# leggedrobotics/art_planner

Hardware: NVIDIA H100
Metric: pose-validity checks/s (higher is better)
Workload: dtype f32

## Files before the change

### art_planner_b200/csrc/artp_capi.cu

```cuda
#include <cassert>
#include <climits>
#include <cmath>
#include <cstdlib>
#include <cstring>
#include <type_traits>
#include <vector>

#include "artp_internal.h"
#include "artp_kernels.cuh"
#include "artp_tiles.cuh"

using namespace artp_api;

namespace {

thread_local std::string g_create_error;

__global__ void reverse_columns_kernel(const float* __restrict__ layer, float* __restrict__ H, int nx, int nz, int pitch) {
  const size_t total = (size_t)pitch * nz;
  for (size_t i = blockIdx.x * (size_t)blockDim.x + threadIdx.x; i < total; i += (size_t)gridDim.x * blockDim.x) {
    const int z = (int)(i / pitch), x = (int)(i - (size_t)z * pitch);
    H[i] = (x < nx) ? layer[x + (size_t)(nz - 1 - z) * nx] * 1.0f + 0.0f : 0.0f;
  }
}

__global__ void build_level_kernel(const float* __restrict__ H, const float2* __restrict__ prevT,
                                   const unsigned char* __restrict__ prevNF, const unsigned char* __restrict__ mergeable,
                                   float2* __restrict__ T, unsigned char* __restrict__ NF, int nx, int nz, int pitch, int half) {
  const size_t total = (size_t)pitch * nz;
  for (size_t i = blockIdx.x * (size_t)blockDim.x + threadIdx.x; i < total; i += (size_t)gridDim.x * blockDim.x) {
    const int z = (int)(i / pitch), x = (int)(i - (size_t)z * pitch);
    if (x >= nx) { T[i] = make_float2(0.f, 0.f); NF[i] = 0; continue; }
    const int x2 = min(x + half, nx - 1), z2 = min(z + half, nz - 1);
    const size_t id[4] = {(size_t)z * pitch + x, (size_t)z * pitch + x2, (size_t)z2 * pitch + x, (size_t)z2 * pitch + x2};
    float mx = -CUDART_INF_F, mn = CUDART_INF_F;
    unsigned char nf = 0;
#pragma unroll
    for (int q = 0; q < 4; ++q) {
      if (prevT) {
        const float2 v = prevT[id[q]];
        mx = fmaxf(mx, v.x); mn = fminf(mn, v.y); nf |= prevNF[id[q]];
      } else {
        const float h = H[id[q]];
        mx = fmaxf(mx, h);
        if (fabsf(h) < CUDART_INF_F) mn = fminf(mn, h); else nf |= 1;
        nf |= mergeable[id[q]];
      }
    }
    T[i] = make_float2(mx, mn);
    NF[i] = nf;
  }
}

__global__ void build_codes_kernel(const float2* __restrict__ T, const unsigned char* __restrict__ NF, uint32_t* __restrict__ C,
                                   size_t n, float base, float step) {
  const float top = artp::code_dec(base, step, artp::kCodeMax);
  for (size_t i = blockIdx.x * (size_t)blockDim.x + threadIdx.x; i < n; i += (size_t)gridDim.x * blockDim.x) {
    const float2 v = T[i];
    uint32_t cM = 0, cm = artp::kCodeNone;
    if (v.x > top) cM = artp::kCodeNone;
    else if (v.x > -CUDART_INF_F) {
      uint32_t lo = 1, hi = artp::kCodeMax;
      while (lo < hi) {
        const uint32_t mid = (lo + hi) >> 1;
        if (artp::code_dec(base, step, mid) >= v.x) hi = mid; else lo = mid + 1;
      }
      cM = lo;
    }
    if (v.y <= top) {
      uint32_t lo = 0, hi = artp::kCodeMax;
      while (lo < hi) {
        const uint32_t mid = (lo + hi + 1) >> 1;
        if (artp::code_dec(base, step, mid) <= v.y) lo = mid; else hi = mid - 1;
      }
      cm = lo;
    }
    C[i] = artp::code_word(cM, cm, NF[i] & 3u);
  }
}

void code_scale(const float* layer, size_t n, float& base, float& step) {
  float lo = HUGE_VALF, hi = -HUGE_VALF;
  for (size_t i = 0; i < n; ++i) {
    const float v = layer[i] * 1.0f + 0.0f;
    if (std::fabs(v) < HUGE_VALF) { lo = std::min(lo, v); hi = std::max(hi, v); }
  }
  base = lo <= hi ? lo : 0.0f;
  int e = -126;
  while (e < 127 && artp::code_dec(base, std::ldexp(1.0f, e), artp::kCodeMax) < hi) ++e;
  step = std::ldexp(1.0f, e);
}

struct PlaneSlot { unsigned long long key; uint32_t lo, hi; };
constexpr unsigned long long kEmptyKey = ~0ull;
__device__ __forceinline__ unsigned long long plane_key(int kx, int kz, int kd) {
  return ((unsigned long long)(uint32_t)(kx & 0xffff) << 48) | ((unsigned long long)(uint32_t)(kz & 0xffff) << 32) | (uint32_t)kd;
}
__device__ __forceinline__ uint32_t plane_slot_hash(unsigned long long k) {
  k ^= k >> 33; k *= 0xff51afd7ed558ccdull; k ^= k >> 33; k *= 0xc4ceb9fe1a85ec53ull; k ^= k >> 33;
  return (uint32_t)k;
}
__global__ void plane_table_clear_kernel(PlaneSlot* tab, size_t cap) {
  for (size_t i = blockIdx.x * (size_t)blockDim.x + threadIdx.x; i < cap; i += (size_t)gridDim.x * blockDim.x) {
    tab[i].key = kEmptyKey; tab[i].lo = 0xffffffffu; tab[i].hi = 0u;
  }
}
__device__ __forceinline__ bool cell_tri_plane(const artp::Field& f, int x, int x_off, int z, int u, float pl[4]) {
  float hA, hB, hC, hD;
  artp::load_cell(f, x, z, hA, hB, hC, hD);
  const bool ok = u == 0 ? (artp::finitef(hA) && artp::finitef(hB) && artp::finitef(hC))
                         : (artp::finitef(hD) && artp::finitef(hB) && artp::finitef(hC));
  if (!ok) return false;
  artp::cell_plane(f, u == 0, x + x_off, z, hA, hB, hC, hD, pl);
  return true;
}
__global__ void plane_table_insert_kernel(const artp::Field f, int x_off, PlaneSlot* tab, uint32_t mask) {
  const size_t ncell = (size_t)(f.nx - 1) * (f.nz - 1);
  for (size_t i = blockIdx.x * (size_t)blockDim.x + threadIdx.x; i < 2 * ncell; i += (size_t)gridDim.x * blockDim.x) {
    const size_t c = i >> 1;
    const int u = (int)(i & 1), z = (int)(c / (f.nx - 1)), x = (int)(c - (size_t)z * (f.nx - 1));
    float pl[4];
    if (!cell_tri_plane(f, x, x_off, z, u, pl)) continue;
    const uint32_t id = (uint32_t)(((size_t)z * f.pitch + x) * 2 + u);
    const unsigned long long key = plane_key(artp::nkey(pl[0]), artp::nkey(pl[2]), artp::dkey(pl[3]));
    uint32_t s = plane_slot_hash(key) & mask;
    for (;;) {
      const unsigned long long old = atomicCAS(&tab[s].key, kEmptyKey, key);
      if (old == kEmptyKey || old == key) {
        if (!(tab[s].lo < id && tab[s].hi > id)) { atomicMin(&tab[s].lo, id); atomicMax(&tab[s].hi, id); }
        break;
      }
      s = (s + 1) & mask;
    }
  }
}
__global__ void plane_table_query_kernel(const artp::Field f, int x_off, const PlaneSlot* __restrict__ tab, uint32_t mask,
                                         unsigned char* __restrict__ mergeable) {
  const size_t ncell = (size_t)(f.nx - 1) * (f.nz - 1);
  for (size_t i = blockIdx.x * (size_t)blockDim.x + threadIdx.x; i < 2 * ncell; i += (size_t)gridDim.x * blockDim.x) {
    const size_t c = i >> 1;
    const int u = (int)(i & 1), z = (int)(c / (f.nx - 1)), x = (int)(c - (size_t)z * (f.nx - 1));
    float pl[4];
    if (!cell_tri_plane(f, x, x_off, z, u, pl)) continue;
    const uint32_t id = (uint32_t)(((size_t)z * f.pitch + x) * 2 + u);
    const float e2 = 2.0f * ARTP_EPS;
    const int kx0 = artp::nkey(pl[0] - e2), kx1 = artp::nkey(pl[0] + e2);
    const int kz0 = artp::nkey(pl[2] - e2), kz1 = artp::nkey(pl[2] + e2);
    const int kd0 = artp::dkey(pl[3] - e2), kd1 = artp::dkey(pl[3] + e2);
    bool dup = false;
    for (int kx = kx0; kx <= kx1 && !dup; ++kx)
      for (int kz = kz0; kz <= kz1 && !dup; ++kz)
        for (int kd = kd0; kd <= kd1 && !dup; ++kd) {
          const unsigned long long key = plane_key(kx, kz, kd);
          uint32_t s = plane_slot_hash(key) & mask;
          for (;;) {
            const unsigned long long k = tab[s].key;
            if (k == kEmptyKey) break;
            if (k == key) { dup = tab[s].lo != id || tab[s].hi != id; break; }
            s = (s + 1) & mask;
          }
        }
    if (dup) mergeable[(size_t)z * f.pitch + x] = 2;
  }
}

__global__ void fill_u8_kernel(uint8_t* p, size_t n, uint8_t v) {
  for (size_t i = blockIdx.x * (size_t)blockDim.x + threadIdx.x; i < n; i += (size_t)gridDim.x * blockDim.x) p[i] = v;
}

constexpr int kCompactBlock = 1024;
template <bool BITS>
__device__ __forceinline__ int mask_at(const uint8_t* __restrict__ valid, size_t i) {
  if (BITS) return (int)((reinterpret_cast<const uint32_t*>(valid)[i >> 5] >> (i & 31)) & 1u);
  return valid[i] != 0;
}
template <bool BITS>
__global__ void compact_count_kernel(const uint8_t* __restrict__ valid, size_t n, uint32_t* __restrict__ counts) {
  const size_t i = (size_t)blockIdx.x * kCompactBlock + threadIdx.x;
  const int v = (i < n) && mask_at<BITS>(valid, i);
  const int c = __syncthreads_count(v);
  if (threadIdx.x == 0) counts[blockIdx.x] = (uint32_t)c;
}
__global__ void compact_scan_kernel(uint32_t* counts, size_t nb, uint32_t* total) {
  __shared__ uint32_t carry;
  __shared__ uint32_t wsum[32];
  if (threadIdx.x == 0) carry = 0;
  __syncthreads();
  for (size_t b0 = 0; b0 < nb; b0 += blockDim.x) {
    const size_t i = b0 + threadIdx.x;
    const uint32_t v = i < nb ? counts[i] : 0u;
    uint32_t x = v;
    const int lane = threadIdx.x & 31, wid = threadIdx.x >> 5;
    for (int o = 1; o < 32; o <<= 1) { const uint32_t y = __shfl_up_sync(0xffffffffu, x, o); if (lane >= o) x += y; }
    if (lane == 31) wsum[wid] = x;
    __syncthreads();
    if (wid == 0) {
      uint32_t s = lane < (int)(blockDim.x >> 5) ? wsum[lane] : 0u;
      for (int o = 1; o < 32; o <<= 1) { const uint32_t y = __shfl_up_sync(0xffffffffu, s, o); if (lane >= o) s += y; }
      wsum[lane] = s;
    }
    __syncthreads();
    const uint32_t before = carry + (wid ? wsum[wid - 1] : 0u) + x - v;
    if (i < nb) counts[i] = before;
    __syncthreads();
    if (threadIdx.x == blockDim.x - 1) carry = before + v;
    __syncthreads();
  }
  if (threadIdx.x == 0) *total = carry;
}
template <bool BITS, typename IndexT>
__global__ void compact_scatter_kernel(const uint8_t* __restrict__ valid, size_t n, int64_t base,
                                       const uint32_t* __restrict__ offsets, IndexT* __restrict__ out) {
  __shared__ uint32_t wsum[32];
  const size_t i = (size_t)blockIdx.x * kCompactBlock + threadIdx.x;
  const int v = (i < n) && mask_at<BITS>(valid, i);
  const unsigned bal = __ballot_sync(0xffffffffu, v);
  const int lane = threadIdx.x & 31, wid = threadIdx.x >> 5;
  if (lane == 0) wsum[wid] = __popc(bal);
  __syncthreads();
  if (wid == 0) {
    uint32_t s = wsum[lane];
    for (int o = 1; o < 32; o <<= 1) { const uint32_t y = __shfl_up_sync(0xffffffffu, s, o); if (lane >= o) s += y; }
    wsum[lane] = s;
  }
  __syncthreads();
  if (v) {
    const uint32_t pos = offsets[blockIdx.x] + (wid ? wsum[wid - 1] : 0u) + __popc(bal & ((1u << lane) - 1u));
    out[pos] = (IndexT)(base + (int64_t)i);
  }
}

__global__ void pack_bits_kernel(const uint8_t* __restrict__ valid, size_t n, uint32_t* __restrict__ bits) {
  const size_t words = (n + 31) / 32;
  const size_t warps = ((size_t)gridDim.x * blockDim.x) >> 5, wid = ((size_t)blockIdx.x * blockDim.x + threadIdx.x) >> 5;
  const int lane = threadIdx.x & 31;
  for (size_t w = wid; w < words; w += warps) {
    const size_t i = w * 32 + lane;
    const unsigned bal = __ballot_sync(0xffffffffu, i < n && valid[i] != 0);
    if (lane == 0) bits[w] = bal;
  }
}

constexpr size_t kChunkItems = 1u << 20;

int ensure_queues(Handle* h, size_t n_items) {
  const size_t need = 5 * std::min(n_items, kChunkItems);
  if (h->recs_cap >= need) return ARTP_OK;
  const size_t cap = std::max<size_t>(need, 1u << 16);
  h->recs_cap = 0;
  size_t had[4] = {0, 0, 0, 0};
  int rc;
  TRY(grow(h, h->d_recs, had[0], cap));
  TRY(grow(h, h->d_recs_f, had[1], cap));
  TRY(grow(h, h->d_recs_g, had[2], cap));
  TRY(grow(h, h->d_defer, had[3], cap));
  h->recs_cap = cap;
  return ARTP_OK;
}

struct HostFeed {
  const char* host;
  char* dev;
  size_t bytes_per_item;
  size_t slice_items;
  float schedule[8];
};
constexpr size_t kScheduleItems = 1u << 18;
constexpr int kPipeReachCtasPerSm = 2;

__global__ void close_slice_kernel(const BoxQueues* round, BoxQueues* slices, int i) {
  const BoxQueues prev = i ? slices[i - 1] : BoxQueues{};
  slices[i].group = {round->group.end, prev.group.end};
  slices[i].reach = {round->reach.end, prev.reach.end};
  slices[i].big = {round->big.end, prev.big.end};
}

int launch_classify(Handle* h, artp::Work w, size_t lo, size_t hi, cudaStream_t s) {
  w.item_base = (uint32_t)lo;
  w.n_items = (uint32_t)hi;
  BoxQueues* q = &h->d_ctr->q;
  return launch(h, artp::classify_items_kernel, (unsigned)((hi - lo + artp::kClassifyItems - 1) / artp::kClassifyItems),
                artp::kClassifyItems, 0, s, h->chk, w, h->d_recs, h->d_recs_f, h->group_grid ? h->d_recs_g : nullptr, &q->big.end,
                &q->reach.end, &q->group.end, h->mode == 1);
}

int launch_big_tile(Handle* h, artp::Work w, size_t lo, size_t hi, BoxQueues* q, cudaStream_t s) {
  w.item_base = (uint32_t)lo;
  w.n_items = (uint32_t)hi;
  const int wpc = h->tile_warps[0];
  const unsigned grid = (unsigned)std::min<size_t>((size_t)h->tile_grid[0], (5 * (hi - lo) + wpc - 1) / wpc);
  return launch(h, artp::box_tiles_warp_kernel, grid, wpc * 32, h->tile_smem[0], s, h->chk, h->tile_map[0][0], h->tile_map[0][1],
                h->tile_cfg[0], w, h->d_recs, &q->big.end, &q->big.claim, &h->d_ctr->defer, h->d_defer, 0u, h->mode == 1);
}
int launch_reach_warp(Handle* h, artp::Work w, size_t lo, size_t hi, BoxQueues* q, cudaStream_t s, unsigned reach_cap) {
  if (!h->chk.reach_tw) return ARTP_OK;
  w.item_base = (uint32_t)lo;
  w.n_items = (uint32_t)hi;
  const int wpc = h->tile_warps[1];
  const unsigned grid = (unsigned)std::min<size_t>({(size_t)h->tile_grid[1], (4 * (hi - lo) + wpc - 1) / wpc, reach_cap});
  return launch(h, artp::box_tiles_warp_kernel, grid, wpc * 32, h->tile_smem[1], s, h->chk, h->tile_map[1][1], h->tile_map[1][1],
                h->tile_cfg[1], w, h->d_recs_f, &q->reach.end, &q->reach.claim, &h->d_ctr->defer, h->d_defer, artp::kDeferReachBit,
                h->mode == 1);
}
int launch_reach_groups(Handle* h, artp::Work w, size_t lo, size_t hi, BoxQueues* q, cudaStream_t s, unsigned reach_cap) {
  if (!h->group_grid) return ARTP_OK;
  w.item_base = (uint32_t)lo;
  w.n_items = (uint32_t)hi;
  const unsigned grid = (unsigned)std::min<size_t>({(size_t)h->group_grid, (hi - lo + 7) / 8, reach_cap});
  return launch(h, artp::reach_groups_kernel, grid, artp::kMaxTileWarps * 32, h->group_smem, s, h->chk, h->tile_map[1][1],
                h->tile_cfg[1], w, h->d_recs_g, &q->group.end, &q->group.claim);
}

int launch_grouping(Handle* h, artp::Work w, size_t lo, size_t hi, cudaStream_t s) {
  w.item_base = (uint32_t)lo;
  w.n_items = (uint32_t)hi;
  const unsigned grid = (unsigned)std::min<size_t>((size_t)h->k2_grid, 5 * (hi - lo));
  return launch(h, artp::box_items_block_kernel, grid, artp::kBlockStageThreads, h->k2_smem, s, h->chk, w, h->d_recs, h->d_recs_f,
                &h->d_ctr->defer, h->d_defer, h->k2_tcap, h->d_err);
}

int run_round_device(Handle* h, const artp::Work& w, cudaStream_t s, size_t base, size_t end, bool timed) {
  CU_TRY(h, cudaMemsetAsync(h->d_ctr, 0, sizeof(Counters), s));
  if (timed) CU_TRY(h, cudaEventRecord(h->ev[0], s));
  TRY(launch_classify(h, w, base, end, s));
  if (timed) CU_TRY(h, cudaEventRecord(h->ev[1], s));
  const bool fork = !h->timing && h->chk.reach_tw;
  if (fork) {
    CU_TRY(h, cudaEventRecord(h->slice_ev[0], s));
    CU_TRY(h, cudaStreamWaitEvent(h->box_stream, h->slice_ev[0], 0));
    if (h->group_grid) CU_TRY(h, cudaStreamWaitEvent(h->group_stream, h->slice_ev[0], 0));
  }
  BoxQueues* q = &h->d_ctr->q;
  TRY(launch_big_tile(h, w, base, end, q, s));
  if (timed) CU_TRY(h, cudaEventRecord(h->ev[2], s));
  TRY(launch_reach_warp(h, w, base, end, q, fork ? h->box_stream : s, UINT_MAX));
  if (timed) CU_TRY(h, cudaEventRecord(h->ev[3], s));
  TRY(launch_reach_groups(h, w, base, end, q, fork ? h->group_stream : s, UINT_MAX));
  if (fork) {
    CU_TRY(h, cudaEventRecord(h->box_ev, h->box_stream));
    CU_TRY(h, cudaStreamWaitEvent(s, h->box_ev, 0));
    if (h->group_grid) {
      CU_TRY(h, cudaEventRecord(h->group_ev, h->group_stream));
      CU_TRY(h, cudaStreamWaitEvent(s, h->group_ev, 0));
    }
  }
  if (timed) CU_TRY(h, cudaEventRecord(h->ev[4], s));
  TRY(launch_grouping(h, w, base, end, s));
  if (timed) { CU_TRY(h, cudaEventRecord(h->ev[5], s)); h->ev_valid = true; }
  return ARTP_OK;
}

int run_round_piped(Handle* h, const artp::Work& w, cudaStream_t s, const HostFeed& feed, size_t base, size_t end) {
  size_t cut[kMaxSlices + 1];
  int ncut = 0;
  cut[0] = base;
  if (end - base >= kScheduleItems) {
    double acc = 0.0;
    for (int i = 0; i < 8 && feed.schedule[i] > 0.0f; ++i) {
      acc += feed.schedule[i];
      const size_t c = std::min(end, (base + (size_t)((double)(end - base) * acc) + 127) & ~(size_t)127);
      if (c > cut[ncut]) cut[++ncut] = c;
    }
    if (cut[ncut] != end) cut[++ncut] = end;
  } else {
    for (size_t lo = base; lo < end; lo += feed.slice_items) cut[++ncut] = std::min(end, lo + feed.slice_items);
  }
  assert(ncut <= kMaxSlices);
  CU_TRY(h, cudaMemsetAsync(h->d_ctr, 0, sizeof(Counters), s));
  const unsigned reach_cap = (unsigned)(kPipeReachCtasPerSm * h->sm_count);
  for (int si = 0; si < ncut; ++si) {
    const size_t lo = cut[si], hi = cut[si + 1];
    CU_TRY(h, cudaMemcpyAsync(feed.dev + lo * feed.bytes_per_item, feed.host + lo * feed.bytes_per_item,
                              (hi - lo) * feed.bytes_per_item, cudaMemcpyHostToDevice, h->copy_stream));
    CU_TRY(h, cudaEventRecord(h->copy_ev[si], h->copy_stream));
    CU_TRY(h, cudaStreamWaitEvent(s, h->copy_ev[si], 0));
    TRY(launch_classify(h, w, lo, hi, s));
    TRY(launch(h, close_slice_kernel, 1, 1, 0, s, &h->d_ctr->q, h->d_slices, si));
    CU_TRY(h, cudaEventRecord(h->slice_ev[si], s));
    CU_TRY(h, cudaStreamWaitEvent(h->box_stream, h->slice_ev[si], 0));
    if (h->group_grid) CU_TRY(h, cudaStreamWaitEvent(h->group_stream, h->slice_ev[si], 0));
    TRY(launch_reach_groups(h, w, lo, hi, h->d_slices + si, h->group_stream, reach_cap));
    TRY(launch_reach_warp(h, w, lo, hi, h->d_slices + si, h->box_stream, reach_cap));
    TRY(launch_big_tile(h, w, lo, hi, h->d_slices + si, h->box_stream));
  }
  if (h->group_grid) {
    CU_TRY(h, cudaEventRecord(h->group_ev, h->group_stream));
    CU_TRY(h, cudaStreamWaitEvent(h->box_stream, h->group_ev, 0));
  }
  TRY(launch_grouping(h, w, base, end, h->box_stream));
  CU_TRY(h, cudaEventRecord(h->box_ev, h->box_stream));
  CU_TRY(h, cudaStreamWaitEvent(s, h->box_ev, 0));
  return ARTP_OK;
}

int run_items(Handle* h, artp::Work w, cudaStream_t s, const HostFeed* feed = nullptr) {
  const size_t n_total = w.n_items;
  TRY(ensure_queues(h, n_total));
  for (size_t base = 0; base < n_total; base += kChunkItems) {
    const size_t end = std::min(n_total, base + kChunkItems);
    if (feed && feed->slice_items < end - base && !h->timing) {
      TRY(run_round_piped(h, w, s, *feed, base, end));
    } else {
      if (feed)
        CU_TRY(h, cudaMemcpyAsync(feed->dev + base * feed->bytes_per_item, feed->host + base * feed->bytes_per_item,
                                  (end - base) * feed->bytes_per_item, cudaMemcpyHostToDevice, s));
      TRY(run_round_device(h, w, s, base, end, h->timing && end == n_total));
    }
  }
  h->deferred_unread = true;
  return ARTP_OK;
}

int check_common(Handle* h, size_t n) {
  TRY(require_map(h));
  if (n >= (size_t)0xFFFFFFF0u) { h->err = "too many items for one call"; return ARTP_E_LIMIT; }
  return ARTP_OK;
}

int check_poses_small(Handle* h, const artp::SmallBatch& sb, size_t n, uint8_t* valid, int steps = -1) {
  TRY(host_call_begin(h));
  if (!h->h_small_out) {
    CU_TRY(h, cudaHostAlloc((void**)&h->h_small_out, 64, cudaHostAllocMapped));
    CU_TRY(h, cudaFuncSetAttribute(artp::pose_small_kernel, cudaFuncAttributeMaxDynamicSharedMemorySize, 200 * 1024));
  }
  uint8_t* d_out = nullptr;
  CU_TRY(h, cudaHostGetDevicePointer((void**)&d_out, h->h_small_out, 0));
  TRY(launch(h, artp::pose_small_kernel, (unsigned)n, 256, h->k2_smem, h->stream, h->chk, sb, d_out, h->k2_tcap, h->d_err,
      h->mode == 1, steps));
  const int rc = host_call_end(h, true);
  if (rc == ARTP_E_CUDA) return rc;
  if (steps < 0) {
    std::memcpy(valid, h->h_small_out, n);
  } else {
    const size_t per = (size_t)steps + 1;
    for (size_t e = 0; e < n / per; ++e) {
      uint8_t ok = 1;
      for (size_t j = 0; j < per; ++j) ok &= h->h_small_out[e * per + j];
      valid[e] = ok;
    }
  }
  h->stats.poses_checked += n;
  h->ev_valid = false;
  return rc;
}

template <typename T>
int check_states(Handle* h, const T* d_states, size_t n, uint8_t* d_valid, cudaStream_t s, const HostFeed* feed = nullptr) {
  artp::Work w;
  if constexpr (std::is_same_v<T, float>) w.s2f = d_states; else w.s2 = d_states;
  w.valid = d_valid;
  w.n_items = (uint32_t)n;
  TRY(run_items(h, w, s, feed));
  h->stats.poses_checked += n;
  return ARTP_OK;
}

template <typename T>
int check_poses(Handle* h, const T* states, size_t n, uint8_t* valid, bool on_device, cudaStream_t stream) {
  TRY(check_common(h, n));
  if (n == 0) return ARTP_OK;
  if (!states || !valid) return null_buffer(h);
  if (on_device) {
    CU_TRY(h, cudaSetDevice(h->device));
    ChainScope cs(h, 0, stream);
    if (cs.rc) return cs.rc;
    return check_states(h, states, n, valid, stream);
  }
  if (n <= (size_t)artp::kSmallBatch && !h->timing) {
    artp::SmallBatch sb;
    for (size_t i = 0; i < n * 7; ++i) (&sb.s[0][0])[i] = (double)states[i];
    return check_poses_small(h, sb, n, valid);
  }
  char* r[2];
  TRY(host_call_begin(h, {n * 7 * sizeof(T), n}, r));
  const HostFeed feed = std::is_same_v<T, float>
                            ? HostFeed{(const char*)states, r[0], 7 * sizeof(T), 256 * 1024, {0.08f, 0.17f, 0.25f, 0.25f, 0.25f}}
                            : HostFeed{(const char*)states, r[0], 7 * sizeof(T), 128 * 1024, {0.06f, 0.14f, 0.20f, 0.20f, 0.20f, 0.20f}};
  TRY(check_states(h, (const T*)r[0], n, (uint8_t*)r[1], h->stream, &feed));
  CU_TRY(h, cudaMemcpyAsync(valid, r[1], n, cudaMemcpyDeviceToHost, h->stream));
  return host_call_end(h, true);
}

int motion_items(Handle* h, size_t n, int n_steps) {
  if (n_steps < 0) { h->err = "n_steps < 0"; return ARTP_E_INVALID; }
  return check_common(h, n * ((size_t)n_steps + 1));
}
int check_motions_on(Handle* h, const double* d_s1, const double* d_s2, size_t n, int n_steps, uint8_t* d_valid, cudaStream_t s) {
  TRY(launch(h, fill_u8_kernel, grid_for(h, n, 256, 8), 256, 0, s, d_valid, n, 1));
  const size_t items = n * ((size_t)n_steps + 1);
  artp::Work w;
  w.s1 = d_s1; w.s2 = d_s2; w.valid = d_valid; w.n_items = (uint32_t)items; w.steps = n_steps; w.edge_mode = 1;
  TRY(run_items(h, w, s));
  h->stats.poses_checked += items;
  return ARTP_OK;
}

__global__ void edge_prefix_kernel(const uint8_t* __restrict__ item_valid, const uint32_t* __restrict__ item_off, size_t n,
                                   int32_t* __restrict__ valid_prefix) {
  for (size_t e = blockIdx.x * (size_t)blockDim.x + threadIdx.x; e < n; e += (size_t)gridDim.x * blockDim.x) {
    const uint32_t o0 = item_off[e], o1 = item_off[e + 1];
    uint32_t k = o0;
    while (k < o1 && item_valid[k]) ++k;
    valid_prefix[e] = (int32_t)(k - o0);
  }
}

int check_items_prefix(Handle* h, const double* d_s1, const double* d_s2, size_t n, const uint32_t* d_item_off,
                       size_t total_items, uint8_t* d_item_valid, int32_t* d_valid_prefix, void* stream, int quotient) {
  TRY(check_common(h, total_items));
  if (n == 0) return ARTP_OK;
  if (!d_s1 || !d_s2 || !d_item_off || !d_valid_prefix || (total_items && !d_item_valid)) {
    return null_buffer(h);
  }
  if (n >= 0xFFFFFFFFull) { h->err = "too many edges"; return ARTP_E_INVALID; }
  CU_TRY(h, cudaSetDevice(h->device));
  cudaStream_t s = (cudaStream_t)stream;
  ChainScope cs(h, 0, s);
  if (cs.rc) return cs.rc;
  if (total_items) {
    artp::Work w;
    w.s1 = d_s1; w.s2 = d_s2; w.valid = d_item_valid; w.n_items = (uint32_t)total_items;
    w.item_off = d_item_off; w.n_edges = (uint32_t)n; w.quotient = quotient;
    TRY(run_items(h, w, s));
  }
  TRY(launch(h, edge_prefix_kernel, grid_for(h, n, 256, 8), 256, 0, s, d_item_valid, d_item_off, n, d_valid_prefix));
  h->stats.poses_checked += total_items;
  return ARTP_OK;
}

int check_items_prefix_host(Handle* h, const double* s1, const double* s2, const std::vector<uint32_t>& off, int quotient,
                            int32_t* valid_prefix) {
  const size_t n = off.size() - 1, total = off[n], sb = n * 7 * sizeof(double);
  char* r[5];
  TRY(host_call_begin(h, {sb, sb, (n + 1) * sizeof(uint32_t), n * sizeof(int32_t), total}, r));
  CU_TRY(h, cudaMemcpyAsync(r[0], s1, sb, cudaMemcpyHostToDevice, h->stream));
  CU_TRY(h, cudaMemcpyAsync(r[1], s2, sb, cudaMemcpyHostToDevice, h->stream));
  CU_TRY(h, cudaMemcpyAsync(r[2], off.data(), (n + 1) * sizeof(uint32_t), cudaMemcpyHostToDevice, h->stream));
  TRY(check_items_prefix(h, (const double*)r[0], (const double*)r[1], n, (const uint32_t*)r[2], total, (uint8_t*)r[4],
                         (int32_t*)r[3], h->stream, quotient));
  CU_TRY(h, cudaMemcpyAsync(valid_prefix, r[3], n * sizeof(int32_t), cudaMemcpyDeviceToHost, h->stream));
  return host_call_end(h, true);
}

int pack_valid_bits(Handle* h, const uint8_t* d_valid, size_t n, uint32_t* d_bits, cudaStream_t s) {
  if (n == 0) return ARTP_OK;
  if (!d_valid || !d_bits) return null_buffer(h);
  CU_TRY(h, cudaSetDevice(h->device));
  const size_t words = (n + 31) / 32;
  return launch(h, pack_bits_kernel, grid_for(h, words * 32, 256, 8), 256, 0, s, d_valid, n, d_bits);
}

}

int artp_api::take_sticky_error(Handle* h) {
  if (h->h_err && *(volatile uint32_t*)h->h_err) {
    const uint32_t e = *(volatile uint32_t*)h->h_err;
    *(volatile uint32_t*)h->h_err = 0;
    if (e & 2u) {
      h->err = "a box reached outside this handle's map window (artp_set_map_window: route samples to the shard that holds them, "
               "halo >= box half-diagonal + offsets); affected poses were marked invalid";
      return ARTP_E_WINDOW;
    }
    h->err = "plane-grouping stage overflow: a zone exceeded its shared-memory store; affected poses were marked invalid";
    return ARTP_E_LIMIT;
  }
  return ARTP_OK;
}

int artp_api::check_states_f32(Handle* h, const float* d_states, size_t n, uint8_t* d_valid, cudaStream_t s) {
  return check_states(h, d_states, n, d_valid, s);
}

int artp_api::check_states_cta(Handle* h, const double* d_states, const uint32_t* d_count, const uint32_t* d_stop, size_t max_n,
                               uint8_t* d_valid, cudaStream_t s) {
  if (max_n == 0) return ARTP_OK;
  if (!h->pose_states_smem) {
    CU_TRY(h, cudaFuncSetAttribute(artp::pose_states_kernel, cudaFuncAttributeMaxDynamicSharedMemorySize, 200 * 1024));
    h->pose_states_smem = true;
  }
  TRY(launch(h, artp::pose_states_kernel, (unsigned)max_n, 256, h->k2_smem, s, h->chk, d_states, d_count, d_stop, d_valid,
             h->k2_tcap, h->d_err));
  h->ev_valid = false;
  return ARTP_OK;
}

int artp_api::compact_valid(Handle* h, const uint8_t* d_valid, size_t n, int64_t base, void* d_indices, uint32_t* d_count,
                            cudaStream_t s, bool bits, bool u32) {
  if (n == 0) { CU_TRY(h, cudaMemsetAsync(d_count, 0, sizeof(uint32_t), s)); return ARTP_OK; }
  ChainScope cs(h, 1, s);
  if (cs.rc) return cs.rc;
  const size_t nb = (n + kCompactBlock - 1) / kCompactBlock;
  TRY(grow(h, h->d_block_counts, h->block_counts_cap, nb));
  TRY(bits ? launch(h, compact_count_kernel<true>, (unsigned)nb, kCompactBlock, 0, s, d_valid, n, h->d_block_counts)
           : launch(h, compact_count_kernel<false>, (unsigned)nb, kCompactBlock, 0, s, d_valid, n, h->d_block_counts));
  TRY(launch(h, compact_scan_kernel, 1, 1024, 0, s, h->d_block_counts, nb, d_count));
  if (bits)
    return launch(h, compact_scatter_kernel<true, int64_t>, (unsigned)nb, kCompactBlock, 0, s, d_valid, n, base, h->d_block_counts,
                  (int64_t*)d_indices);
  if (u32)
    return launch(h, compact_scatter_kernel<false, uint32_t>, (unsigned)nb, kCompactBlock, 0, s, d_valid, n, base,
                  h->d_block_counts, (uint32_t*)d_indices);
  return launch(h, compact_scatter_kernel<false, int64_t>, (unsigned)nb, kCompactBlock, 0, s, d_valid, n, base, h->d_block_counts,
                (int64_t*)d_indices);
}

extern "C" {

const char* artp_version(void) { return "artp 0.1 sm_90a"; }

const char* artp_last_error(const artp_handle* hh) {
  if (!hh) return g_create_error.c_str();
  return reinterpret_cast<const Handle*>(hh)->err.c_str();
}

int artp_create(const artp_params* params, artp_handle** out) {
  if (!params || !out) { g_create_error = "null argument"; return ARTP_E_INVALID; }
  *out = nullptr;
  int ndev = 0;
  cudaError_t e = cudaGetDeviceCount(&ndev);
  if (e != cudaSuccess || ndev == 0) {
    g_create_error = std::string("no CUDA device: ") + cudaGetErrorString(e);
    return ARTP_E_CUDA;
  }
  if (params->device < 0 || params->device >= ndev) { g_create_error = "bad device ordinal"; return ARTP_E_INVALID; }
  if (!(params->torso_length > 0 && params->torso_width > 0 && params->torso_height > 0 && params->reach_x > 0 &&
        params->reach_y > 0 && params->reach_z > 0)) {
    g_create_error = "box dimensions must be positive";
    return ARTP_E_INVALID;
  }
  Handle* h = new Handle();
  h->p = *params;
  h->device = params->device;
  auto fail = [&](const char* what, cudaError_t ce) {
    g_create_error = std::string(what) + ": " + cudaGetErrorString(ce);
    artp_destroy(reinterpret_cast<artp_handle*>(h));
    return ARTP_E_CUDA;
  };
  if ((e = cudaSetDevice(h->device)) != cudaSuccess) return fail("cudaSetDevice", e);
  cudaDeviceProp prop;
  if ((e = cudaGetDeviceProperties(&prop, h->device)) != cudaSuccess) return fail("cudaGetDeviceProperties", e);
  h->sm_count = prop.multiProcessorCount;
  cudaFuncAttributes fa;
  if ((e = cudaFuncGetAttributes(&fa, artp::box_tiles_warp_kernel)) != cudaSuccess)
    return fail("no usable kernel image (built for sm_90a)", e);
  for (cudaStream_t* st : {&h->stream, &h->copy_stream, &h->box_stream, &h->group_stream})
    if ((e = cudaStreamCreateWithFlags(st, cudaStreamNonBlocking)) != cudaSuccess) return fail("cudaStreamCreate", e);
  if ((e = cudaEventCreateWithFlags(&h->group_ev, cudaEventDisableTiming)) != cudaSuccess) return fail("cudaEventCreate", e);
  for (int i = 0; i < kMaxSlices; ++i) {
    if ((e = cudaEventCreateWithFlags(&h->copy_ev[i], cudaEventDisableTiming)) != cudaSuccess) return fail("cudaEventCreate", e);
    if ((e = cudaEventCreateWithFlags(&h->slice_ev[i], cudaEventDisableTiming)) != cudaSuccess) return fail("cudaEventCreate", e);
  }
  if ((e = cudaEventCreateWithFlags(&h->box_ev, cudaEventDisableTiming)) != cudaSuccess) return fail("cudaEventCreate", e);
  if ((e = cudaMalloc(&h->d_slices, kMaxSlices * sizeof(BoxQueues))) != cudaSuccess) return fail("cudaMalloc", e);
  if ((e = cudaMalloc(&h->d_ctr, sizeof(Counters))) != cudaSuccess) return fail("cudaMalloc", e);
  for (int g = 0; g < 2; ++g)
    if ((e = cudaEventCreateWithFlags(&h->chain_ev[g], cudaEventDisableTiming)) != cudaSuccess) return fail("cudaEventCreate", e);
  if ((e = cudaHostAlloc((void**)&h->h_err, 64, cudaHostAllocMapped)) != cudaSuccess) return fail("cudaHostAlloc", e);
  *h->h_err = 0;
  if ((e = cudaHostGetDevicePointer((void**)&h->d_err, h->h_err, 0)) != cudaSuccess) return fail("cudaHostGetDevicePointer", e);
  h->cnn = artp_cnn::create(h->device, h->sm_count);
  artp::Checker& c = h->chk;
  std::memset(&c, 0, sizeof(c));
  c.side[0][0] = (float)params->torso_length; c.side[0][1] = (float)params->torso_width; c.side[0][2] = (float)params->torso_height;
  c.side[1][0] = (float)params->reach_x; c.side[1][1] = (float)params->reach_y; c.side[1][2] = (float)params->reach_z;
  c.torso_off[0] = (float)params->torso_off_x; c.torso_off[1] = (float)params->torso_off_y;
  c.torso_off[2] = (float)(params->torso_off_z - params->feet_off_z);
  c.feet_ox = (float)params->feet_off_x; c.feet_oy = (float)params->feet_off_y;
  c.unknown_untraversable = params->unknown_space_untraversable ? 1 : 0;
  *out = reinterpret_cast<artp_handle*>(h);
  return ARTP_OK;
}

void artp_destroy(artp_handle* hh) {
  if (!hh) return;
  Handle* h = reinterpret_cast<Handle*>(hh);
  cudaSetDevice(h->device);
  if (h->stream) { cudaStreamSynchronize(h->stream); cudaStreamDestroy(h->stream); }
  if (h->copy_stream) { cudaStreamSynchronize(h->copy_stream); cudaStreamDestroy(h->copy_stream); }
  if (h->box_stream) { cudaStreamSynchronize(h->box_stream); cudaStreamDestroy(h->box_stream); }
  if (h->group_stream) { cudaStreamSynchronize(h->group_stream); cudaStreamDestroy(h->group_stream); }
  if (h->group_ev) cudaEventDestroy(h->group_ev);
  for (int i = 0; i < kMaxSlices; ++i) {
    if (h->copy_ev[i]) cudaEventDestroy(h->copy_ev[i]);
    if (h->slice_ev[i]) cudaEventDestroy(h->slice_ev[i]);
  }
  if (h->box_ev) cudaEventDestroy(h->box_ev);
  cudaFree(h->d_slices);
  for (int k = 0; k < 2; ++k) for (int l = 0; l <= artp::kMaxLevel; ++l) { cudaFree(h->d_T[k][l]); cudaFree(h->d_C[k][l]); }
  cudaFree(h->d_H[0]); cudaFree(h->d_H[1]); cudaFree(h->d_ctr); cudaFree(h->d_defer); cudaFree(h->d_stage);
  cudaFree(h->d_block_counts); cudaFree(h->d_recs); cudaFree(h->d_recs_f); cudaFree(h->d_recs_g); cudaFree(h->d_samp_layers); cudaFree(h->d_samp_scratch);
  cudaFree(h->d_dist_layers); cudaFree(h->d_dist_scratch); cudaFree(h->d_basic_keep);
  roadmap_free(h);
  if (h->h_small_out) cudaFreeHost(h->h_small_out);
  if (h->h_err) cudaFreeHost(h->h_err);
  for (int g = 0; g < 2; ++g) if (h->chain_ev[g]) cudaEventDestroy(h->chain_ev[g]);
  artp_cnn::destroy(h->cnn);
  for (int i = 0; i < 6; ++i) if (h->ev[i]) cudaEventDestroy(h->ev[i]);
  delete h;
}

int artp_has_map(const artp_handle* hh) {
  if (!hh) return 0;
  Handle* h = reinterpret_cast<Handle*>(const_cast<artp_handle*>(hh));
  std::lock_guard<std::mutex> lock(h->mtx);
  return h->has_map ? 1 : 0;
}

int artp_set_mode(artp_handle* hh, int mode) {
  LOCK_HANDLE(h, hh);
// ... 422 lines not shown
```

Measured before the change: 1.832 billion.

## Route device-resident rounds through sliced path with capped big-tile grid on main stream

Non-timing rounds now all go through one sliced routine, including rounds with no host feed. Those rounds use a single slice, skip the close-slice kernel and run big-tile on the main stream. That big-tile grid is capped at one CTA per SM, so it can run at the same time as the reach-warp and reach-group kernels on their side streams. The aim is to overlap the big-tile stage with the reach stages instead of running big-tile first. The cost is fewer CTAs for big-tile, and the speedup depends on how these kernels share SMs.

```diff
diff --git a/art_planner_b200/csrc/artp_capi.cu b/art_planner_b200/csrc/artp_capi.cu
--- a/art_planner_b200/csrc/artp_capi.cu
+++ b/art_planner_b200/csrc/artp_capi.cu
@@ -267,6 +267,7 @@
 };
 constexpr size_t kScheduleItems = 1u << 18;
 constexpr int kPipeReachCtasPerSm = 2;
+constexpr int kOneSliceBigCtasPerSm = 1;
 
 __global__ void close_slice_kernel(const BoxQueues* round, BoxQueues* slices, int i) {
   const BoxQueues prev = i ? slices[i - 1] : BoxQueues{};
@@ -284,11 +285,11 @@
                 &q->reach.end, &q->group.end, h->mode == 1);
 }
 
-int launch_big_tile(Handle* h, artp::Work w, size_t lo, size_t hi, BoxQueues* q, cudaStream_t s) {
+int launch_big_tile(Handle* h, artp::Work w, size_t lo, size_t hi, BoxQueues* q, cudaStream_t s, unsigned big_cap = UINT_MAX) {
   w.item_base = (uint32_t)lo;
   w.n_items = (uint32_t)hi;
   const int wpc = h->tile_warps[0];
-  const unsigned grid = (unsigned)std::min<size_t>((size_t)h->tile_grid[0], (5 * (hi - lo) + wpc - 1) / wpc);
+  const unsigned grid = (unsigned)std::min<size_t>({(size_t)h->tile_grid[0], (5 * (hi - lo) + wpc - 1) / wpc, big_cap});
   return launch(h, artp::box_tiles_warp_kernel, grid, wpc * 32, h->tile_smem[0], s, h->chk, h->tile_map[0][0], h->tile_map[0][1],
                 h->tile_cfg[0], w, h->d_recs, &q->big.end, &q->big.claim, &h->d_ctr->defer, h->d_defer, 0u, h->mode == 1);
 }
@@ -319,77 +320,80 @@
                 &h->d_ctr->defer, h->d_defer, h->k2_tcap, h->d_err);
 }
 
-int run_round_device(Handle* h, const artp::Work& w, cudaStream_t s, size_t base, size_t end, bool timed) {
+int run_round_serial(Handle* h, const artp::Work& w, cudaStream_t s, size_t base, size_t end, bool timed) {
   CU_TRY(h, cudaMemsetAsync(h->d_ctr, 0, sizeof(Counters), s));
   if (timed) CU_TRY(h, cudaEventRecord(h->ev[0], s));
   TRY(launch_classify(h, w, base, end, s));
   if (timed) CU_TRY(h, cudaEventRecord(h->ev[1], s));
-  const bool fork = !h->timing && h->chk.reach_tw;
-  if (fork) {
-    CU_TRY(h, cudaEventRecord(h->slice_ev[0], s));
-    CU_TRY(h, cudaStreamWaitEvent(h->box_stream, h->slice_ev[0], 0));
-    if (h->group_grid) CU_TRY(h, cudaStreamWaitEvent(h->group_stream, h->slice_ev[0], 0));
-  }
   BoxQueues* q = &h->d_ctr->q;
   TRY(launch_big_tile(h, w, base, end, q, s));
   if (timed) CU_TRY(h, cudaEventRecord(h->ev[2], s));
-  TRY(launch_reach_warp(h, w, base, end, q, fork ? h->box_stream : s, UINT_MAX));
+  TRY(launch_reach_warp(h, w, base, end, q, s, UINT_MAX));
   if (timed) CU_TRY(h, cudaEventRecord(h->ev[3], s));
-  TRY(launch_reach_groups(h, w, base, end, q, fork ? h->group_stream : s, UINT_MAX));
-  if (fork) {
-    CU_TRY(h, cudaEventRecord(h->box_ev, h->box_stream));
-    CU_TRY(h, cudaStreamWaitEvent(s, h->box_ev, 0));
-    if (h->group_grid) {
-      CU_TRY(h, cudaEventRecord(h->group_ev, h->group_stream));
-      CU_TRY(h, cudaStreamWaitEvent(s, h->group_ev, 0));
-    }
-  }
+  TRY(launch_reach_groups(h, w, base, end, q, s, UINT_MAX));
   if (timed) CU_TRY(h, cudaEventRecord(h->ev[4], s));
   TRY(launch_grouping(h, w, base, end, s));
   if (timed) { CU_TRY(h, cudaEventRecord(h->ev[5], s)); h->ev_valid = true; }
   return ARTP_OK;
 }
 
-int run_round_piped(Handle* h, const artp::Work& w, cudaStream_t s, const HostFeed& feed, size_t base, size_t end) {
+int run_round_sliced(Handle* h, const artp::Work& w, cudaStream_t s, const HostFeed* feed, size_t base, size_t end) {
   size_t cut[kMaxSlices + 1];
   int ncut = 0;
   cut[0] = base;
-  if (end - base >= kScheduleItems) {
+  if (!feed) {
+    cut[++ncut] = end;
+  } else if (end - base >= kScheduleItems) {
     double acc = 0.0;
-    for (int i = 0; i < 8 && feed.schedule[i] > 0.0f; ++i) {
-      acc += feed.schedule[i];
+    for (int i = 0; i < 8 && feed->schedule[i] > 0.0f; ++i) {
+      acc += feed->schedule[i];
       const size_t c = std::min(end, (base + (size_t)((double)(end - base) * acc) + 127) & ~(size_t)127);
       if (c > cut[ncut]) cut[++ncut] = c;
     }
     if (cut[ncut] != end) cut[++ncut] = end;
   } else {
-    for (size_t lo = base; lo < end; lo += feed.slice_items) cut[++ncut] = std::min(end, lo + feed.slice_items);
+    for (size_t lo = base; lo < end; lo += feed->slice_items) cut[++ncut] = std::min(end, lo + feed->slice_items);
   }
   assert(ncut <= kMaxSlices);
+  const bool one = ncut == 1;
   CU_TRY(h, cudaMemsetAsync(h->d_ctr, 0, sizeof(Counters), s));
-  const unsigned reach_cap = (unsigned)(kPipeReachCtasPerSm * h->sm_count);
+  const unsigned reach_cap = one ? UINT_MAX : (unsigned)(kPipeReachCtasPerSm * h->sm_count);
   for (int si = 0; si < ncut; ++si) {
     const size_t lo = cut[si], hi = cut[si + 1];
-    CU_TRY(h, cudaMemcpyAsync(feed.dev + lo * feed.bytes_per_item, feed.host + lo * feed.bytes_per_item,
-                              (hi - lo) * feed.bytes_per_item, cudaMemcpyHostToDevice, h->copy_stream));
-    CU_TRY(h, cudaEventRecord(h->copy_ev[si], h->copy_stream));
-    CU_TRY(h, cudaStreamWaitEvent(s, h->copy_ev[si], 0));
+    if (feed) {
+      CU_TRY(h, cudaMemcpyAsync(feed->dev + lo * feed->bytes_per_item, feed->host + lo * feed->bytes_per_item,
+                                (hi - lo) * feed->bytes_per_item, cudaMemcpyHostToDevice, h->copy_stream));
+      CU_TRY(h, cudaEventRecord(h->copy_ev[si], h->copy_stream));
+      CU_TRY(h, cudaStreamWaitEvent(s, h->copy_ev[si], 0));
+    }
     TRY(launch_classify(h, w, lo, hi, s));
-    TRY(launch(h, close_slice_kernel, 1, 1, 0, s, &h->d_ctr->q, h->d_slices, si));
+    BoxQueues* q = &h->d_ctr->q;
+    if (!one) {
+      TRY(launch(h, close_slice_kernel, 1, 1, 0, s, &h->d_ctr->q, h->d_slices, si));
+      q = h->d_slices + si;
+    }
     CU_TRY(h, cudaEventRecord(h->slice_ev[si], s));
     CU_TRY(h, cudaStreamWaitEvent(h->box_stream, h->slice_ev[si], 0));
     if (h->group_grid) CU_TRY(h, cudaStreamWaitEvent(h->group_stream, h->slice_ev[si], 0));
-    TRY(launch_reach_groups(h, w, lo, hi, h->d_slices + si, h->group_stream, reach_cap));
-    TRY(launch_reach_warp(h, w, lo, hi, h->d_slices + si, h->box_stream, reach_cap));
-    TRY(launch_big_tile(h, w, lo, hi, h->d_slices + si, h->box_stream));
+    TRY(launch_reach_groups(h, w, lo, hi, q, h->group_stream, reach_cap));
+    TRY(launch_reach_warp(h, w, lo, hi, q, h->box_stream, reach_cap));
+    if (one) TRY(launch_big_tile(h, w, lo, hi, q, s, (unsigned)(kOneSliceBigCtasPerSm * h->sm_count)));
+    else TRY(launch_big_tile(h, w, lo, hi, q, h->box_stream));
+  }
+  cudaStream_t gs = one ? s : h->box_stream;
+  if (one) {
+    CU_TRY(h, cudaEventRecord(h->box_ev, h->box_stream));
+    CU_TRY(h, cudaStreamWaitEvent(s, h->box_ev, 0));
   }
   if (h->group_grid) {
     CU_TRY(h, cudaEventRecord(h->group_ev, h->group_stream));
-    CU_TRY(h, cudaStreamWaitEvent(h->box_stream, h->group_ev, 0));
-  }
-  TRY(launch_grouping(h, w, base, end, h->box_stream));
-  CU_TRY(h, cudaEventRecord(h->box_ev, h->box_stream));
-  CU_TRY(h, cudaStreamWaitEvent(s, h->box_ev, 0));
+    CU_TRY(h, cudaStreamWaitEvent(gs, h->group_ev, 0));
+  }
+  TRY(launch_grouping(h, w, base, end, gs));
+  if (!one) {
+    CU_TRY(h, cudaEventRecord(h->box_ev, h->box_stream));
+    CU_TRY(h, cudaStreamWaitEvent(s, h->box_ev, 0));
+  }
   return ARTP_OK;
 }
 
@@ -398,13 +402,13 @@
   TRY(ensure_queues(h, n_total));
   for (size_t base = 0; base < n_total; base += kChunkItems) {
     const size_t end = std::min(n_total, base + kChunkItems);
-    if (feed && feed->slice_items < end - base && !h->timing) {
-      TRY(run_round_piped(h, w, s, *feed, base, end));
+    if (!h->timing) {
+      TRY(run_round_sliced(h, w, s, feed, base, end));
     } else {
       if (feed)
         CU_TRY(h, cudaMemcpyAsync(feed->dev + base * feed->bytes_per_item, feed->host + base * feed->bytes_per_item,
                                   (end - base) * feed->bytes_per_item, cudaMemcpyHostToDevice, s));
-      TRY(run_round_device(h, w, s, base, end, h->timing && end == n_total));
+      TRY(run_round_serial(h, w, s, base, end, end == n_total));
     }
   }
   h->deferred_unread = true;
```

Result: no change. 1.832 billion, median of 6 (+0.0%).
